# LemonATsu/DANBO-pytorch

Hardware: AMD Instinct MI355X
Metric: ray-samples/sec at 512x512x64 samples (higher is better)
Workload: dtype f32 (fp16x2-split MFMA products, fp32 accumulate); 1 GPU; H36M danbo_base network, 512x512 rays x (48 coarse + 16 importance) samples, 1 pose / 1 camera per rank, cylinder near/far, exact in-volume culling; rays=262144, samples_per_ray=64, parallelism=rays-dp1

## Files before the change

### danbo-pytorch_amd/core/_hip.py

```python
import ctypes
import os
import re
from ctypes import c_char_p, c_float, c_int, c_void_p
from types import SimpleNamespace

import torch

_HERE = os.path.dirname(os.path.abspath(__file__))
LIB_PATH = os.environ.get("DANBO_HIP_LIB") or os.path.join(os.path.dirname(_HERE), "libdanbo_hip.so")

P = c_void_p
I = c_int
F = c_float


class HeaderError(ValueError):
    """include/danbo_hip.h left the subset of C that parse_header reads"""


_SCALARS = {"int": c_int, "long": ctypes.c_long, "long long": ctypes.c_longlong, "size_t": ctypes.c_size_t, "float": c_float,
            **{f"{u}int{n}_t": getattr(ctypes, f"c_{u}int{n}") for u in ("", "u") for n in (8, 16, 32, 64)}}
_TAIL = r"((?:\*\s*(?:const\b\s*)?)*)(\w+)\s*(?:\[\s*(\w*)\s*\])?$"
_DECL = re.compile(r"(?:const\s+)?(long\s+long|\w+)\b\s*" + _TAIL)
_MORE = re.compile(_TAIL)
# ... 177 lines not shown
    _p_functions, _p_structs, _p_constants = parse_header(_f.read())
if _p_structs or _p_constants or set(_p_functions) & (set(_functions) | set(_r_functions)):
    raise HeaderError(f"{PARTMAP_HEADER_PATH} declares a struct, a constant, or a name another header declares")
PARTMAP_SIGNATURES = {name: argtypes for name, (_, argtypes) in _p_functions.items()}
PARTMAP_RESTYPES = {name: restype for name, (restype, _) in _p_functions.items()}

METRICS_HEADER_PATH = os.path.join(os.path.dirname(HEADER_PATH), "danbo_metrics.h")
if not os.path.exists(METRICS_HEADER_PATH):
    raise RuntimeError(f"{METRICS_HEADER_PATH} not found (the binding of the image metrics is derived from it, it lies beside danbo_hip.h)")
with open(METRICS_HEADER_PATH) as _f:
    _m_functions, _m_structs, _m_constants = parse_header(_f.read())
if _m_structs or _m_constants or set(_m_functions) & (set(_functions) | set(_r_functions) | set(_p_functions)):
    raise HeaderError(f"{METRICS_HEADER_PATH} declares a struct, a constant, or a name another header declares")
METRICS_SIGNATURES = {name: argtypes for name, (_, argtypes) in _m_functions.items()}
METRICS_RESTYPES = {name: restype for name, (restype, _) in _m_functions.items()}
ANERF_MAX_D = C.DANBO_ANERF_MAX_D

TRAIN_TENSORS = (
    ["graph_net.layers.0.lin.weight", "graph_net.layers.0.adj_w", "graph_net.layers.0.bias", "graph_net.layers.1.lin.weight",
     "graph_net.layers.1.adj_w", "graph_net.layers.1.bias", "graph_net.layers.2.weight", "graph_net.layers.2.bias",
     "graph_net.layers.3.weight", "graph_net.layers.3.bias", "graph_net.axis_scale",
     "prob_linears.layers.0.lin.weight", "prob_linears.layers.0.adj_w", "prob_linears.layers.0.bias", "prob_linears.layers.1.weight",
     "prob_linears.layers.1.bias", "prob_linears.layers.2.weight", "prob_linears.layers.2.bias"]
    + [f"pts_linears.{i}.weight" for i in range(8)] + [f"pts_linears.{i}.bias" for i in range(8)]
    + ["alpha_linear.weight", "alpha_linear.bias", "feature_linear.weight", "feature_linear.bias", "views_linears.0.weight",
       "views_linears.0.bias", "rgb_linear.weight", "rgb_linear.bias", "framecodes.codes.weight"])
N_TRAIN_TENSORS = C.DANBO_T_COUNT
_anchors = {"graph_net.axis_scale": C.DANBO_T_AXIS_SCALE, "prob_linears.layers.0.lin.weight": C.DANBO_T_A_W0,
            "pts_linears.0.weight": C.DANBO_T_PTS_W0, "pts_linears.0.bias": C.DANBO_T_PTS_B0, "alpha_linear.weight": C.DANBO_T_ALPHA_W,
            "framecodes.codes.weight": C.DANBO_T_CODES}
if len(TRAIN_TENSORS) != N_TRAIN_TENSORS or any(TRAIN_TENSORS.index(k) != i for k, i in _anchors.items()):
    raise HeaderError(f"TRAIN_TENSORS does not line up with enum DanboTrainTensor of {HEADER_PATH}")

_lib = None


def lib():
    global _lib
    if _lib is None:
        if not os.path.exists(LIB_PATH):
            raise RuntimeError(
                f"{LIB_PATH} not found: build it with `make -C danbo-pytorch_amd/csrc` "
                "(or __graft_entry__.build()).  There is no CPU / PyTorch fallback.")
        l = ctypes.CDLL(LIB_PATH)
        for name, argtypes in {**SIGNATURES, **RASTER_SIGNATURES, **PARTMAP_SIGNATURES, **METRICS_SIGNATURES}.items():
            fn = getattr(l, name)
            fn.argtypes = argtypes
            fn.restype = RESTYPES.get(name) or RASTER_RESTYPES.get(name) or PARTMAP_RESTYPES.get(name) or METRICS_RESTYPES[name]
        if l.danbo_abi_version() != C.DANBO_ABI_VERSION:
            raise RuntimeError(f"{LIB_PATH} has ABI version {l.danbo_abi_version()}, {HEADER_PATH} declares {C.DANBO_ABI_VERSION}: "
                               "the library is stale, rebuild it with `make -C danbo-pytorch_amd/csrc`")
        _lib = l
    return _lib


def ptr(t):
    return None if t is None else c_void_p(t.data_ptr())


def stream():
    return c_void_p(torch.cuda.current_stream().cuda_stream)


# ... 12 lines not shown
```

### danbo-pytorch_amd/core/hip_ops.py

```python
import ctypes

import torch

from . import _hip
from ._hip import call as _call, ptr as _p, stream as _stream

J = _hip.C.DANBO_J
VOL = _hip.C.DANBO_VOL
FEAT = _hip.C.DANBO_FEAT
RAY_FLAT_VMAX = _hip.C.DANBO_RAY_FLAT_VMAX
H_STRIDE = _hip.C.DANBO_H_STRIDE
MLP_PACKED_FLOATS = _hip.C.DANBO_MLP_PACKED_FLOATS
ASSIGN16_PACKED_BYTES = _hip.C.DANBO_ASSIGN16_PACKED_BYTES
MLP16_PACKED_BYTES = _hip.C.DANBO_MLP16_PACKED_BYTES
ANERF_ENC_FLOATS = _hip.C.DANBO_ANERF_ENC_FLOATS
LINEAR16_ENC_K = _hip.C.DANBO_LINEAR16_ENC_K
TRUNK_PACKED_BYTES = _hip.C.DANBO_TRUNK_PACKED_BYTES
TRUNK_PE_WIDTH = _hip.C.DANBO_TRUNK_PE_WIDTH
VIEW_W = 128


def _f32(t, name):
    if t is None:
        return None
# ... 78 lines not shown


def bone_cull(geo, compact=True, cnt=None):
    bits = torch.empty(geo.M, device=geo.device, dtype=torch.int32)
    lst = None
    if compact:
        lst = torch.empty(geo.M, device=geo.device, dtype=torch.int32)
        if cnt is None:
            cnt = torch.zeros(1, device=geo.device, dtype=torch.int32)
        assert cnt.dtype == torch.int32 and cnt.numel() == 1 and cnt.is_contiguous()
    else:
        cnt = None
    rm = tuple(geo.ray_mask) if geo.ray_mask is not None else (None, None, None)
    flat = rm[3] if len(rm) > 3 else None
    _call("danbo_bone_cull", *geo.head(), _p(rm[0]), _p(rm[1]), _p(rm[2]), _p(flat), _p(bits), _p(lst), _p(cnt), _stream())
    return bits, lst, cnt


def ray_bone_mask(rays_o, rays_d, skts, align, axis_scale, t_lo, t_hi, want_flat=False):
    rays_o, rays_d, skts = _f32(rays_o, "rays_o"), _f32(rays_d, "rays_d"), _f32(skts, "skts")
    t_lo, t_hi = _f32(t_lo, "t_lo").reshape(-1), _f32(t_hi, "t_hi").reshape(-1)
    R, G = rays_o.shape[0], skts.shape[0]
    assert t_lo.shape[0] == R and t_hi.shape[0] == R
    mask = torch.empty(R, device=rays_o.device, dtype=torch.int32)
    flat = torch.empty(R, device=rays_o.device, dtype=torch.int32) if want_flat else None
    _call("danbo_ray_bone_mask", _p(rays_o), _p(rays_d), _p(t_lo), _p(t_hi), R, G, _p(skts), _p(_f32(align, "align")),
          _p(_f32(axis_scale, "axis_scale")), _p(mask), _p(flat), _stream())
    return (mask, t_lo, t_hi, flat) if want_flat else (mask, t_lo, t_hi)


# ... 781 lines not shown
```

### danbo-pytorch_amd/core/render_engine.py

```python
import ctypes

import torch

from . import _hip
from . import hip_ops as ops


class RenderEngine:
    fuse_resample = False

    def _key(self):
        return tuple((k, v.data_ptr(), v._version) for k, v in sorted(self.p.items()))

    def _sampling(self, N_samples, N_importance):
        cfg = self.cfg
        return (N_samples or cfg["N_samples"], N_importance or cfg["N_importance"], cfg["density_scale"],
                ops.density_act(cfg.get("density_act")))

    @staticmethod
    def frame_result(out, out0):
        return dict(rgb_map=out["rgb_map"], disp_map=out["disp_map"], acc_map=out["acc_map"], alpha=out["alpha"],
                    T_i=out["weights"], rgb0=out0["rgb_map"], disp0=out0["disp_map"], acc0=out0["acc_map"],
                    alpha0=out0["alpha"])

# ... 59 lines not shown
    fuse_resample = True

    def __init__(self, cfg, params, align, buffers=None, mlp_mode="f16split"):
        self.cfg = cfg
        self.p = params
        self.align = align.float().contiguous()
        self._packed_key = None
        self.packed = self.wrt = self.empty_consts = None
        self.mean_code = None
        self.profile = None
        self.skip_flat_rays = True
        self.mlp_form = 32
        assert mlp_mode in ("f16split", "fp32")
        self.mlp_mode = mlp_mode
        self.group_rows = False

    def refresh(self):
        key = self._key()
        if key == self._packed_key and getattr(self, "_built_mode", None) == (self.mlp_mode, self.mlp_form):
            return
        p = self.p
        dev = p["alpha_linear.weight"].device
        q = self._equalized(p) if self.mlp_mode == "f16split" else p
        self.pts_w = [q[f"pts_linears.{i}.weight"] for i in range(8)]
        self.pts_b = [q[f"pts_linears.{i}.bias"].contiguous() for i in range(8)]
        self.packed, self.wrt = ops.mlp_pack(self.pts_w, q["feature_linear.weight"], q["views_linears.0.weight"])
        self.packed16, self.views_b16 = ops.mlp16_pack(self.pts_w, q["feature_linear.weight"],
                                                       q["feature_linear.bias"], q["views_linears.0.weight"],
                                                       q["views_linears.0.bias"], form=self.mlp_form)
        self.alpha_w = q["alpha_linear.weight"].reshape(-1).contiguous()
# ... 106 lines not shown
        self.refresh()
        return ops.pose_volumes(bones, self.gw, self.cfg["multires_graph"])

    def view_constants(self, rays_d, skts, cam_idx, ray_list=None, ray_count=None):
        self.refresh()
        cfg = self.cfg
        ray_mode = {"world": 0, "root_local": 1}[cfg["ray_tr_type"]]
        normalise = 1 if cfg["view_type"] == "relray" else 0
        return ops.view_consts(rays_d, skts, ray_mode, normalise, cfg["multires_views"], self.framecodes,
                               self.mean_code, cam_idx, self.wrt,
                               self.views_b16 if self.mlp_mode == "f16split" else self.views_b, self.rgb_w,
                               self.rgb_b, self.empty_consts, {16: 1, 32: 2}[self.mlp_form] if self.mlp_mode == "f16split" else 0,
                               self.code_table, ray_list, ray_count)

    def forward_samples(self, rays_o, rays_d, skts, bones, cam_idx=None, z=None, pts=None, dense=False,
                        want_confd=False, volumes=None, view=None, fill=True, ray_mask=None, count=None):
        self.refresh()
        geo = ops.Geometry(rays_o, rays_d, skts, self.align, self.axis_scale, z=z, pts=pts, ray_mask=ray_mask)
        vols = self.volumes(bones) if volumes is None else volumes
        cview, raw_empty = self.view_constants(geo.rays_d, geo.skts, cam_idx) if view is None else view
        S = geo.S
        bits, lst, cnt = ops.bone_cull(geo, compact=not dense, cnt=count)
        if lst is not None and self.mlp_mode == "f16split" and self.group_rows:
            ops.group_rows(bits, lst, cnt)
        if self.mlp_mode == "f16split":
            h, confd = ops.gather_assign_blend16(geo, vols, bits, self.aw, self.assign16, lst, cnt, geo.M, want_confd)
        else:
            h, confd = ops.gather_assign_blend(geo, vols, bits, self.aw, lst, cnt, geo.M, want_confd)
        raw = ops.fill_raw(raw_empty, S) if fill or dense else torch.empty(geo.R, S, 4, device=raw_empty.device)
        if self.profile is not None:
            e0, e1 = torch.cuda.Event(enable_timing=True), torch.cuda.Event(enable_timing=True)
            e0.record()
        self._mlp(h, S, cview, raw, lst, cnt, geo.M)
        if self.profile is not None:
            e1.record()
            self.profile.setdefault("k_pe_mlp", []).append((e0, e1, cnt if cnt is not None else geo.M))
        extras = dict(valid_bits=bits, list=lst, count=cnt, confd_rows=confd, h_rows=h, volumes=vols)
# ... 78 lines not shown
            ops.near_far_boxes(rays_o, rays_d, skts, self.align, self.axis_scale, near, far)
        return near, far

    def render(self, rays_o, rays_d, skts, bones, cyls, cam_idx=None, N_samples=None, N_importance=None,
               chunk=4096, near_far=None, dense=False, keep=False, part_map=None, part_valid_only=False):
        S, Sf, B, act = self._sampling(N_samples, N_importance)
        self.refresh()
        part = self._part_mode(part_map)
        if part and not self._part_exact_culled(act):
            dense = True
        fused = S <= 64 and Sf <= 64
        lazy = not dense and not keep
        flat_mode = (lazy and (fused or (S <= 256 and Sf <= 64)) and self.skip_flat_rays and self.flat_rays_ok
                     and act[0] == "relu")
        near, far = self.near_far(rays_o, rays_d, cyls, skts, 0.0, 1.0, chunk) if near_far is None else near_far
        z = ops.coarse_samples(near, far, S)
        ray_mask = None if dense else ops.ray_bone_mask(rays_o, rays_d, skts, self.align, self.axis_scale, near, far,
                                                        want_flat=flat_mode)
        counts = torch.zeros(3, device=rays_o.device, dtype=torch.int32)
        flat = None
        vols = self.volumes(bones)
        if flat_mode:
            flat = ops.flat_rays(ray_mask[1], ray_mask[3], S, Sf, want_weights=not fused or bool(part), cnt=counts[2:3])
            view = self.view_constants(rays_d, skts, cam_idx, flat["ray_list"], flat["ray_count"])
        else:
            view = self.view_constants(rays_d, skts, cam_idx)
        if ray_mask is not None:
            ray_mask = ray_mask[:3]
        raw, ex = self.forward_samples(rays_o, rays_d, skts, bones, cam_idx, z=z, dense=dense, volumes=vols, view=view,
                                       fill=not lazy, ray_mask=ray_mask, count=counts[0:1], want_confd=bool(part))
        if fused:
            out0, z_all, z_fine, order = ops.composite_importance(
                raw, z, rays_d, Sf, B, bits=ex["valid_bits"] if lazy else None, raw_empty=view[1] if lazy else None,
                want_weights=keep or bool(part), flat=flat, act=act)
        else:
            out0 = ops.composite(raw, z, rays_d, B, bits=ex["valid_bits"] if lazy else None, raw_empty=view[1] if lazy else None,
                                 flat=flat, act=act)
            z_all, z_fine, order = ops.importance_samples(z, out0["weights"], Sf, flat=flat)
        raw_f, ex_f = self.forward_samples(rays_o, rays_d, skts, bones, cam_idx, z=z_fine, dense=dense,
                                           volumes=vols, view=view, fill=not lazy,
                                           ray_mask=ray_mask, count=counts[1:2], want_confd=bool(part))
        out = ops.composite_merged(raw, raw_f, order, z_all, rays_d, B, bits_a=ex["valid_bits"] if lazy else None,
                                   bits_b=ex_f["valid_bits"] if lazy else None, raw_empty=view[1] if lazy else None,
                                   want_raw=keep, flat=flat, act=act)
        if part:
            col, cb = self._part_colors(ex, S, part, part_valid_only, dense)
            col_f, cb_f = self._part_colors(ex_f, Sf, part, part_valid_only, dense)
            ops.composite_colors(col, out0["weights"], bits_a=cb, flat=flat, out=out0["rgb_map"])
            ops.composite_colors(col, out["weights"], col_f, order, cb, cb_f, flat=flat, out=out["rgb_map"])
        ret = self.frame_result(out, out0)
        if keep:
            ret.update(near=near, far=far, z_coarse=z, raw_coarse=raw, weights_coarse=out0["weights"], z_fine=z_fine,
                       z_sorted=z_all, sorted_idxs=order, raw_fine=raw_f, raw_sorted=out.get("raw_sorted"),
                       count_coarse=ex["count"], count_fine=ex_f["count"], valid_bits=ex["valid_bits"])
            if part:
                ret.update(confd_coarse=ex["confd_rows"], confd_fine=ex_f["confd_rows"], list_coarse=ex["list"],
# ... 14 lines not shown
```

### danbo-pytorch_amd/csrc/k_frame.hip

```cpp
#include "common.hpp"

using namespace danbo;

namespace {
struct FrameBuffers {
    float *near, *far, *cyl_scratch, *z, *vol_scratch, *volumes, *cview, *raw_empty, *h, *raw_a, *raw_b, *z_fine, *z_sorted, *weights0;
    uint32_t *bits_a, *bits_b, *ray_mask, *ray_flat;
    int32_t *list, *count, *order, *ray_list;
};

FrameBuffers carve(Carver& c, int R, int G, int S, int Sf, int chunk, int Wg) {
    FrameBuffers b;
    const size_t M = (size_t)R * S, Mf = (size_t)R * Sf;
    b.near = c.take<float>(R);
    b.far = c.take<float>(R);
    b.cyl_scratch = c.take<float>(8 * (size_t)((R + chunk - 1) / chunk));
    b.z = c.take<float>(M);
    b.vol_scratch = c.take<float>(3 * (size_t)G * 24 * Wg);
    b.volumes = c.take<float>((size_t)G * 24 * 240);
    b.cview = c.take<float>((size_t)R * 128);
    b.raw_empty = c.take<float>((size_t)R * 4);
    b.ray_mask = c.take<uint32_t>(R);
    b.ray_flat = c.take<uint32_t>(R);
    b.ray_list = c.take<int32_t>(R);
// ... 25 lines not shown
    DANBO_CHECK_ARG(m && r && o && workspace && S >= 3 && S <= 256 && Sf >= 1 && Sf <= 64);
    DANBO_CHECK_ARG(r->R >= 1 && r->G >= 1 && r->R % r->G == 0 && r->chunk >= 1);
    DANBO_CHECK_ARG(r->rays_o && r->rays_d && r->skts && r->bones && r->cyls);
    DANBO_CHECK_ARG(o->rgb_map && o->disp_map && o->acc_map && o->alpha && o->weights && o->rgb0 && o->disp0 && o->acc0 && o->alpha0);
    const int R = r->R, G = r->G;
    const bool flat_rays = m->flat_rays_ok != 0 && act == DANBO_DENSITY_RELU;
    DANBO_CHECK_ARG(workspace_bytes >= danbo_render_frame_workspace(R, G, S, Sf, r->chunk, m->graph_width));
    Carver c(workspace);
    const FrameBuffers b = carve(c, R, G, S, Sf, r->chunk, m->graph_width);
    hipStream_t st = (hipStream_t)stream;

    DANBO_TRY(danbo_near_far_cylinder(r->rays_o, r->rays_d, r->cyls, R, G, 0.f, 1.f, r->near_in, r->far_in, r->chunk, b.cyl_scratch,
                                      b.near, b.far, stream));
    if (m->use_volume_near_far)
        DANBO_TRY(danbo_near_far_boxes(r->rays_o, r->rays_d, r->skts, m->align, m->axis_scale, R, G, b.near, b.far, stream));
    DANBO_TRY(danbo_coarse_samples(b.near, b.far, R, S, nullptr, b.z, stream));
    DANBO_TRY(danbo_ray_bone_mask(r->rays_o, r->rays_d, b.near, b.far, R, G, r->skts, m->align, m->axis_scale, b.ray_mask,
                                  flat_rays ? b.ray_flat : nullptr, stream));
    DANBO_TRY(danbo_pose_volumes_fwd(r->bones, G, m->L_graph, m->graph_width, m->g_w0, m->g_adjw0, m->g_b0, m->g_w1, m->g_adjw1, m->g_b1,
                                     m->g_w2, m->g_b2, m->g_w3, m->g_b3, b.vol_scratch, b.volumes, stream));
    zero_words(b.count, 4, nullptr, 0, st);
    auto view_consts = [&](const int32_t* ray_list, const int32_t* ray_count) -> int {
        return danbo_view_consts(r->rays_d, r->skts, R, G, m->ray_mode, m->normalise, m->L_view, m->framecodes, m->n_codes, m->code_size,
                                 m->mean_code, r->cam_idx, m->views_w_ray_t, m->views_b_eff, m->rgb_w, m->rgb_b, m->empty_consts, 2,
                                 m->code_table, ray_list, ray_count, b.cview, b.raw_empty, stream);
    };
    const int32_t *ray_list = nullptr, *ray_count = nullptr;
    if (flat_rays) {
        DANBO_TRY(danbo_flat_rays(b.near, b.ray_flat, R, S, Sf, o->rgb0, o->disp0, o->acc0, b.weights0, o->alpha0, b.z_fine, o->rgb_map,
                                  o->disp_map, o->acc_map, o->weights, o->alpha, b.ray_list, b.count + 3, 3, stream));
        ray_list = b.ray_list;
        ray_count = b.count + 3;
    }
    DANBO_TRY(view_consts(ray_list, ray_count));
    auto cull = [&](const float* zz, int s, uint32_t* bits, int32_t* count) -> int {
        DANBO_TRY(danbo_bone_cull(r->rays_o, r->rays_d, zz, nullptr, R, s, G, r->skts, m->align, m->axis_scale, b.ray_mask, b.near, b.far,
                                  nullptr, bits, b.list, count, stream));
        return 0;
    };
    auto network = [&](const float* zz, int s, uint32_t* bits, int32_t* count, float* raw) -> int {
        DANBO_TRY(danbo_gather_assign_blend16_fwd(r->rays_o, r->rays_d, zz, nullptr, R, s, G, r->skts, m->align, m->axis_scale, b.volumes,
                                                  bits, b.list, count, R * s, m->assign16, m->a_b0, m->a_b1, m->a_w2, m->a_b2, b.h,
                                                  nullptr, reinterpret_cast<uint32_t*>(b.count + 2), stream));
        return danbo_pe_mlp32_fwd(b.h, b.list, count, R * s, s, m->mlp16, m->pts_b, m->alpha_w, m->alpha_b, b.cview, m->rgb_w,
                                  m->rgb_b, raw, nullptr, stream);
    };
    DANBO_TRY(cull(b.z, S, b.bits_a, b.count));
    DANBO_TRY(network(b.z, S, b.bits_a, b.count, b.raw_a));
    if (S <= 64) {
        DANBO_TRY(danbo_composite_importance_pdf_fwd_act(b.raw_a, b.raw_empty, b.bits_a, b.z, r->rays_d, R, S, Sf, m->density_scale, nullptr,
// ... 26 lines not shown
```

### danbo-pytorch_amd/csrc/k_sample.hip

```cpp
#include "common.hpp"

namespace danbo {

__global__ __launch_bounds__(256) DANBO_NO_PK_F32 void k_cylinder_pass1(const float* __restrict__ rays_o,
                                                        const float* __restrict__ rays_d,
                                                        const float* __restrict__ cyl, int R, int G,
                                                        float near0, float far0,
                                                        const float* __restrict__ near_in,
                                                        const float* __restrict__ far_in, int chunk,
                                                        double* __restrict__ acc,
                                                        float* __restrict__ near_out,
                                                        float* __restrict__ far_out) {
    const int rays_per_pose = R / G;
    for (int r0 = blockIdx.x * blockDim.x; r0 < R; r0 += gridDim.x * blockDim.x) {
        const int r = r0 + threadIdx.x;
        const bool act = r < R;
        const int rc = act ? r : R - 1;
        const int g = min(rc / rays_per_pose, G - 1);
        float o[3] = {rays_o[3 * rc], rays_o[3 * rc + 1], rays_o[3 * rc + 2]};
        float d[3] = {rays_d[3 * rc], rays_d[3 * rc + 1], rays_d[3 * rc + 2]};
        float c[3] = {cyl[5 * g], cyl[5 * g + 1], cyl[5 * g + 2]};
        float nr, fr;
        const bool hit = cylinder_bounds(o, d, c, near_in ? near_in[rc] : near0, far_in ? far_in[rc] : far0, &nr, &fr) && act;
        if (act) {
// ... 131 lines not shown
        }
        int any = ok ? 1 : 0;
#pragma unroll
        for (int off = 16; off > 0; off >>= 1) {
            lo = fminf(lo, __shfl_xor(lo, off, 64));
            hi = fmaxf(hi, __shfl_xor(hi, off, 64));
            any |= __shfl_xor(any, off, 64);
        }
        if (j == 0 && r0 < R && any) {
            near_io[r] = lo;
            far_io[r] = hi;
        }
    }
}

__device__ __forceinline__ float coarse_sample(float n_, float f_, int s, int S, const float* __restrict__ t_rand, long m) {
    float v = coarse_z(n_, f_, s, S);
    if (t_rand) {
        const float zp = s > 0 ? coarse_z(n_, f_, s - 1, S) : v;
        const float zn = s + 1 < S ? coarse_z(n_, f_, s + 1, S) : v;
        const float lower = s > 0 ? mul_rn(0.5f, add_rn(v, zp)) : v;
        const float upper = s + 1 < S ? mul_rn(0.5f, add_rn(zn, v)) : v;
        v = add_rn(lower, mul_rn(sub_rn(upper, lower), t_rand[m]));
    }
    return v;
}

__global__ __launch_bounds__(256) void k_coarse_samples4(const float* __restrict__ nr, const float* __restrict__ fr,
                                                         int R, int S, const float* __restrict__ t_rand,
                                                         float4* __restrict__ z) {
    const unsigned S4 = (unsigned)S / 4u;
    const unsigned M4 = (unsigned)R * S4;
    for (unsigned q = blockIdx.x * blockDim.x + threadIdx.x; q < M4; q += gridDim.x * blockDim.x) {
        const unsigned r = q / S4;
        const int s0 = 4 * (int)(q - r * S4);
        const float n_ = nr[r], f_ = fr[r];
        const long m = 4L * q;
        float4 v;
        v.x = coarse_sample(n_, f_, s0, S, t_rand, m);
        v.y = coarse_sample(n_, f_, s0 + 1, S, t_rand, m + 1);
        v.z = coarse_sample(n_, f_, s0 + 2, S, t_rand, m + 2);
        v.w = coarse_sample(n_, f_, s0 + 3, S, t_rand, m + 3);
// ... 20 lines not shown
}

__device__ __forceinline__ void load_point(const float* __restrict__ rays_o, const float* __restrict__ rays_d,
                                           const float* __restrict__ z, const float* __restrict__ pts, long m, int S,
                                           float* p) {
    if (pts != nullptr) {
        p[0] = pts[3 * m]; p[1] = pts[3 * m + 1]; p[2] = pts[3 * m + 2];
    } else {
        const int r = (int)(m / S);
        const float o[3] = {rays_o[3 * r], rays_o[3 * r + 1], rays_o[3 * r + 2]};
        const float d[3] = {rays_d[3 * r], rays_d[3 * r + 1], rays_d[3 * r + 2]};
        sample_point(o, d, z[m], p);
    }
}

typedef float v2f __attribute__((ext_vector_type(2)));

template <int HI>
__device__ __forceinline__ v2f pk_mul_bcast(v2f m, v2f x) {
    v2f d;
    if (HI) asm("v_pk_mul_f32 %0, %1, %2 op_sel:[1,0] op_sel_hi:[1,1]" : "=v"(d) : "v"(m), "v"(x));
    else asm("v_pk_mul_f32 %0, %1, %2 op_sel:[0,0] op_sel_hi:[0,1]" : "=v"(d) : "v"(m), "v"(x));
    return d;
}
__device__ __forceinline__ v2f pk_add(v2f a, v2f b) {
    v2f d;
    asm("v_pk_add_f32 %0, %1, %2" : "=v"(d) : "v"(a), "v"(b));
    return d;
}
__device__ __forceinline__ v2f pk_add_bcast_hi(v2f m, v2f a) {
    v2f d;
    asm("v_pk_add_f32 %0, %1, %2 op_sel:[1,0] op_sel_hi:[1,1]" : "=v"(d) : "v"(m), "v"(a));
    return d;
}
__device__ __forceinline__ void affine_pk(const float* M, v2f x, v2f y, v2f z, v2f* q) {
#pragma unroll
    for (int k = 0; k < 3; ++k) {
        const float4 r = *reinterpret_cast<const float4*>(M + 4 * k);
        const v2f m01 = {r.x, r.y}, m23 = {r.z, r.w};
        v2f s = pk_add(pk_mul_bcast<0>(m01, x), pk_mul_bcast<1>(m01, y));
        s = pk_add(s, pk_mul_bcast<0>(m23, z));
        q[k] = pk_add_bcast_hi(m23, s);
    }
}

__device__ __forceinline__ bool segment_misses_bone(const float* sk, const float* al, const float* sc ,
                                                    const float* o, const float* d, float zl, float zh) {
    float ol[3], dl[3], t[3];
    bone_local(sk, al, o, ol);
    for (int k = 0; k < 3; ++k) t[k] = sk[4 * k] * d[0] + sk[4 * k + 1] * d[1] + sk[4 * k + 2] * d[2];
    for (int k = 0; k < 3; ++k) dl[k] = al[4 * k] * t[0] + al[4 * k + 1] * t[1] + al[4 * k + 2] * t[2];
    const float pad = 1e-4f * fmaxf(fabsf(zl), fabsf(zh)) + 1e-5f;
    float tmin = zl - pad, tmax = zh + pad;
    bool miss = false;
    for (int k = 0; k < 3; ++k) {
        const float s = sc[k] * 1.001f + 1e-4f;
        if (fabsf(dl[k]) < 1e-12f) {
            miss = miss || fabsf(ol[k]) > s;
        } else {
// ... 109 lines not shown
    const bool prefilter = pts == nullptr && ray_mask == nullptr && nrays <= CULL_MAX_RAYS;
    float zreg[CULL_SPT];
    if (pts == nullptr) {
#pragma unroll
        for (int k = 0; k < CULL_SPT; ++k) zreg[k] = z[min(base + k * CULL_BLOCK + threadIdx.x, M - 1)];
    }
    uint32_t pre[CULL_SPT];
    if (ray_mask != nullptr) {
        bool any = false;
#pragma unroll
        for (int k = 0; k < CULL_SPT; ++k) {
            pre[k] = 0u;
            if (base + k * CULL_BLOCK + threadIdx.x < M) {
                const int r = r_first + ray_of(off0 + k * CULL_BLOCK + threadIdx.x);
                const float lo = t_lo[r], hi = t_hi[r];
                const float slack = 5e-5f * fmaxf(fabsf(lo), fabsf(hi));
                const bool inside = zreg[k] >= lo - slack && zreg[k] <= hi + slack;
                pre[k] = inside ? ray_mask[r] : (1u << J) - 1u;
                if (!inside && ray_flat != nullptr) ray_flat[r] = 0u;
            }
            any = any || pre[k] != 0u;
        }
        if (!__syncthreads_or(any ? 1 : 0)) {
#pragma unroll
            for (int k = 0; k < CULL_SPT; ++k)
                if (base + k * CULL_BLOCK + threadIdx.x < M) valid_bits[base + k * CULL_BLOCK + threadIdx.x] = 0u;
            return;
        }
    }
    for (int i = threadIdx.x; i < J * 16; i += CULL_BLOCK) s_align[i] = align[i];
    for (int i = threadIdx.x; i < J * 4; i += CULL_BLOCK) s_scale[i] = (i & 3) < 3 ? fabsf(axis_scale[(i >> 2) * 3 + (i & 3)]) : 0.f;
// ... 55 lines not shown
            sample_point(oa, da, ma < M ? zreg[2 * pr] : z[M - 1], pa);
            sample_point(ob, db, mb < M ? zreg[2 * pr + 1] : z[M - 1], pb);
        }
        const int ga = pose_of(ra), gb = pose_of(rb);
        uint32_t ba = 0, bb = 0;
        uint32_t need = (1u << J) - 1u;
        if (ray_mask != nullptr) {
            need = wave_or(pre[2 * pr] | pre[2 * pr + 1]);
        } else if (prefilter) {
            uint32_t mine = s_mask[ra - r_first] | s_mask[rb - r_first];
            need = wave_or(mine);
        }
        if (__builtin_amdgcn_readfirstlane((int)__all(ga == gb))) {
            const v2f px = {pa[0], pb[0]}, py = {pa[1], pb[1]}, pz = {pa[2], pb[2]};
            const float* sk = s_skt + (ga - g0) * J * 16;
            while (need) {
                const int j = __builtin_ctz(need);
                need &= need - 1u;
                v2f l[3], t[3];
                affine_pk(sk + 16 * j, px, py, pz, l);
                affine_pk(s_align + 16 * j, l[0], l[1], l[2], t);
                const float* sc = s_scale + 4 * j;
                const bool ina = !(fabsf(t[0].x) > sc[0] || fabsf(t[1].x) > sc[1] || fabsf(t[2].x) > sc[2]);
                const bool inb = !(fabsf(t[0].y) > sc[0] || fabsf(t[1].y) > sc[1] || fabsf(t[2].y) > sc[2]);
                ba |= (ina ? 1u : 0u) << j;
                bb |= (inb ? 1u : 0u) << j;
            }
        } else {
            const float* ska = s_skt + (ga - g0) * J * 16;
            const float* skb = s_skt + (gb - g0) * J * 16;
            for (int j = 0; j < J; ++j) {
                float pt[3];
                bone_local(ska + 16 * j, s_align + 16 * j, pa, pt);
                ba |= (in_volume(pt, s_scale + 4 * j) ? 1u : 0u) << j;
                bone_local(skb + 16 * j, s_align + 16 * j, pb, pt);
                bb |= (in_volume(pt, s_scale + 4 * j) ? 1u : 0u) << j;
            }
        }
        bits4[2 * pr] = ma < M ? ba : 0u;
        bits4[2 * pr + 1] = mb < M ? bb : 0u;
        if (ma < M) valid_bits[ma] = ba;
        if (mb < M) valid_bits[mb] = bb;
// ... 927 lines not shown
```

### danbo-pytorch_amd/csrc/sample_math.hpp

```cpp
#pragma once
#include <math.h>
#include <stdint.h>

#if defined(__HIPCC__)
#define DANBO_HD __host__ __device__ __forceinline__
#else
#define DANBO_HD inline
#endif

namespace danbo {

constexpr int J = 24;
constexpr int FEAT = 15;
constexpr int VOXF = 5;
constexpr int VRES = 16;
constexpr int VOL = 240;

#if defined(__HIP_DEVICE_COMPILE__)
DANBO_HD float mul_rn(float a, float b) { return __fmul_rn(a, b); }
DANBO_HD float add_rn(float a, float b) { return __fadd_rn(a, b); }
DANBO_HD float sub_rn(float a, float b) { return __fsub_rn(a, b); }
DANBO_HD float div_rn(float a, float b) { return __fdiv_rn(a, b); }
DANBO_HD double dmul_rn(double a, double b) { return __dmul_rn(a, b); }
DANBO_HD double dadd_rn(double a, double b) { return __dadd_rn(a, b); }
// ... 6 lines not shown
DANBO_HD double dadd_rn(double a, double b) { volatile double r = a + b; return r; }
#endif

DANBO_HD float norm3_torch(float x, float y, float z) { return sqrtf(fmaf(z, z, fmaf(y, y, mul_rn(x, x)))); }
DANBO_HD float norm2_torch(float x, float y) { return sqrtf(fmaf(y, y, mul_rn(x, x))); }

DANBO_HD float linspace01(int i, int n) {
    if (n <= 1) return 0.f;
    const float step = div_rn(1.0f, (float)(n - 1));
    return (i < n / 2) ? mul_rn((float)i, step) : sub_rn(1.0f, mul_rn((float)(n - 1 - i), step));
}

DANBO_HD float coarse_z(float nr, float fr, int s, int S) {
    const float t = linspace01(s, S);
    return add_rn(mul_rn(nr, sub_rn(1.0f, t)), mul_rn(fr, t));
}

DANBO_HD void sample_point(const float* o, const float* d, float z, float* p) {
    p[0] = add_rn(o[0], mul_rn(d[0], z));
    p[1] = add_rn(o[1], mul_rn(d[1], z));
    p[2] = add_rn(o[2], mul_rn(d[2], z));
}

DANBO_HD void rotate_unfused(const float* M, const float* d, float* q) {
#pragma unroll
    for (int k = 0; k < 3; ++k) {
        const float* r = M + 4 * k;
        q[k] = add_rn(add_rn(mul_rn(r[0], d[0]), mul_rn(r[1], d[1])), mul_rn(r[2], d[2]));
    }
}
// ... 253 lines not shown
```

Measured before the change: 3.859 billion ray-samples/s.

## Cull only listed non-flat rays and fuse coarse sampling into the cull

Adds a bone-cull kernel that walks only the compacted list of non-flat rays instead of every ray-sample, and for the coarse pass also generates the z samples inline, so the separate coarse_samples launch is dropped. Per-ray origin, direction and mask data are staged in shared memory, and each workgroup compacts its output list with ballots and a single atomic. The aim is to avoid culling work on flat or empty rays and to save one full pass over z. The catch is that z is left uninitialised for unlisted rays, so downstream consumers must never read those entries. It applies only when there is a single pose and flat-ray mode is on.

```diff
diff --git a/danbo-pytorch_amd/core/_hip.py b/danbo-pytorch_amd/core/_hip.py
--- a/danbo-pytorch_amd/core/_hip.py
+++ b/danbo-pytorch_amd/core/_hip.py
@@ -215,6 +215,16 @@
     raise HeaderError(f"{METRICS_HEADER_PATH} declares a struct, a constant, or a name another header declares")
 METRICS_SIGNATURES = {name: argtypes for name, (_, argtypes) in _m_functions.items()}
 METRICS_RESTYPES = {name: restype for name, (restype, _) in _m_functions.items()}
+
+CULL_HEADER_PATH = os.path.join(os.path.dirname(HEADER_PATH), "danbo_cull.h")
+if not os.path.exists(CULL_HEADER_PATH):
+    raise RuntimeError(f"{CULL_HEADER_PATH} not found (the binding of the listed-ray cull is derived from it, it lies beside danbo_hip.h)")
+with open(CULL_HEADER_PATH) as _f:
+    _c_functions, _c_structs, _c_constants = parse_header(_f.read())
+if _c_structs or _c_constants or set(_c_functions) & (set(_functions) | set(_r_functions) | set(_p_functions) | set(_m_functions)):
+    raise HeaderError(f"{CULL_HEADER_PATH} declares a struct, a constant, or a name another header declares")
+CULL_SIGNATURES = {name: argtypes for name, (_, argtypes) in _c_functions.items()}
+CULL_RESTYPES = {name: restype for name, (restype, _) in _c_functions.items()}
 ANERF_MAX_D = C.DANBO_ANERF_MAX_D
 
 TRAIN_TENSORS = (
@@ -244,10 +254,11 @@
                 f"{LIB_PATH} not found: build it with `make -C danbo-pytorch_amd/csrc` "
                 "(or __graft_entry__.build()).  There is no CPU / PyTorch fallback.")
         l = ctypes.CDLL(LIB_PATH)
-        for name, argtypes in {**SIGNATURES, **RASTER_SIGNATURES, **PARTMAP_SIGNATURES, **METRICS_SIGNATURES}.items():
+        for name, argtypes in {**SIGNATURES, **RASTER_SIGNATURES, **PARTMAP_SIGNATURES, **METRICS_SIGNATURES, **CULL_SIGNATURES}.items():
             fn = getattr(l, name)
             fn.argtypes = argtypes
-            fn.restype = RESTYPES.get(name) or RASTER_RESTYPES.get(name) or PARTMAP_RESTYPES.get(name) or METRICS_RESTYPES[name]
+            fn.restype = (RESTYPES.get(name) or RASTER_RESTYPES.get(name) or PARTMAP_RESTYPES.get(name) or METRICS_RESTYPES.get(name)
+                          or CULL_RESTYPES[name])
         if l.danbo_abi_version() != C.DANBO_ABI_VERSION:
             raise RuntimeError(f"{LIB_PATH} has ABI version {l.danbo_abi_version()}, {HEADER_PATH} declares {C.DANBO_ABI_VERSION}: "
                                "the library is stale, rebuild it with `make -C danbo-pytorch_amd/csrc`")
diff --git a/danbo-pytorch_amd/core/hip_ops.py b/danbo-pytorch_amd/core/hip_ops.py
--- a/danbo-pytorch_amd/core/hip_ops.py
+++ b/danbo-pytorch_amd/core/hip_ops.py
@@ -116,6 +116,22 @@
     rm = tuple(geo.ray_mask) if geo.ray_mask is not None else (None, None, None)
     flat = rm[3] if len(rm) > 3 else None
     _call("danbo_bone_cull", *geo.head(), _p(rm[0]), _p(rm[1]), _p(rm[2]), _p(flat), _p(bits), _p(lst), _p(cnt), _stream())
+    return bits, lst, cnt
+
+
+def bone_cull_rays(geo, flat, bounds=None, cnt=None, rays_per_wg=0):
+    assert geo.z is not None and geo.ray_mask is not None and geo.z.is_contiguous()
+    bits = torch.empty(geo.M, device=geo.device, dtype=torch.int32)
+    lst = torch.empty(geo.M, device=geo.device, dtype=torch.int32)
+    if cnt is None:
+        cnt = torch.zeros(1, device=geo.device, dtype=torch.int32)
+    assert cnt.dtype == torch.int32 and cnt.numel() == 1 and cnt.is_contiguous()
+    near, far = (None, None) if bounds is None else (_f32(b, "bounds").reshape(-1) for b in bounds)
+    assert near is None or (near.shape[0] == geo.R and far.shape[0] == geo.R)
+    rm = tuple(geo.ray_mask)
+    _call("danbo_bone_cull_rays", *_ray_list(flat), _p(rm[0]), _p(rm[1]), _p(rm[2]), _p(geo.rays_o), _p(geo.rays_d), geo.R, geo.S,
+          geo.G, _p(geo.skts), _p(geo.align), _p(geo.axis_scale), _p(near), _p(far), _p(geo.z), int(rays_per_wg), _p(bits), _p(lst),
+          _p(cnt), _stream())
     return bits, lst, cnt
 
 
diff --git a/danbo-pytorch_amd/core/render_engine.py b/danbo-pytorch_amd/core/render_engine.py
--- a/danbo-pytorch_amd/core/render_engine.py
+++ b/danbo-pytorch_amd/core/render_engine.py
@@ -97,6 +97,7 @@
         assert mlp_mode in ("f16split", "fp32")
         self.mlp_mode = mlp_mode
         self.group_rows = False
+        self.cull_listed_rays = True
 
     def refresh(self):
         key = self._key()
@@ -233,13 +234,17 @@
                                self.code_table, ray_list, ray_count)
 
     def forward_samples(self, rays_o, rays_d, skts, bones, cam_idx=None, z=None, pts=None, dense=False,
-                        want_confd=False, volumes=None, view=None, fill=True, ray_mask=None, count=None):
+                        want_confd=False, volumes=None, view=None, fill=True, ray_mask=None, count=None, listed=None):
         self.refresh()
         geo = ops.Geometry(rays_o, rays_d, skts, self.align, self.axis_scale, z=z, pts=pts, ray_mask=ray_mask)
         vols = self.volumes(bones) if volumes is None else volumes
         cview, raw_empty = self.view_constants(geo.rays_d, geo.skts, cam_idx) if view is None else view
         S = geo.S
-        bits, lst, cnt = ops.bone_cull(geo, compact=not dense, cnt=count)
+        if listed is not None:
+            assert not dense and pts is None
+            bits, lst, cnt = ops.bone_cull_rays(geo, listed[0], listed[1], cnt=count)
+        else:
+            bits, lst, cnt = ops.bone_cull(geo, compact=not dense, cnt=count)
         if lst is not None and self.mlp_mode == "f16split" and self.group_rows:
             ops.group_rows(bits, lst, cnt)
         if self.mlp_mode == "f16split":
@@ -348,7 +353,8 @@
         flat_mode = (lazy and (fused or (S <= 256 and Sf <= 64)) and self.skip_flat_rays and self.flat_rays_ok
                      and act[0] == "relu")
         near, far = self.near_far(rays_o, rays_d, cyls, skts, 0.0, 1.0, chunk) if near_far is None else near_far
-        z = ops.coarse_samples(near, far, S)
+        listed_cull = flat_mode and self.cull_listed_rays and not part and skts.shape[0] == 1
+        z = torch.empty(rays_o.shape[0], S, device=rays_o.device, dtype=torch.float32) if listed_cull else ops.coarse_samples(near, far, S)
         ray_mask = None if dense else ops.ray_bone_mask(rays_o, rays_d, skts, self.align, self.axis_scale, near, far,
                                                         want_flat=flat_mode)
         counts = torch.zeros(3, device=rays_o.device, dtype=torch.int32)
@@ -362,7 +368,8 @@
         if ray_mask is not None:
             ray_mask = ray_mask[:3]
         raw, ex = self.forward_samples(rays_o, rays_d, skts, bones, cam_idx, z=z, dense=dense, volumes=vols, view=view,
-                                       fill=not lazy, ray_mask=ray_mask, count=counts[0:1], want_confd=bool(part))
+                                       fill=not lazy, ray_mask=ray_mask, count=counts[0:1], want_confd=bool(part),
+                                       listed=(flat, (near, far)) if listed_cull else None)
         if fused:
             out0, z_all, z_fine, order = ops.composite_importance(
                 raw, z, rays_d, Sf, B, bits=ex["valid_bits"] if lazy else None, raw_empty=view[1] if lazy else None,
@@ -373,7 +380,8 @@
             z_all, z_fine, order = ops.importance_samples(z, out0["weights"], Sf, flat=flat)
         raw_f, ex_f = self.forward_samples(rays_o, rays_d, skts, bones, cam_idx, z=z_fine, dense=dense,
                                            volumes=vols, view=view, fill=not lazy,
-                                           ray_mask=ray_mask, count=counts[1:2], want_confd=bool(part))
+                                           ray_mask=ray_mask, count=counts[1:2], want_confd=bool(part),
+                                           listed=(flat, None) if listed_cull else None)
         out = ops.composite_merged(raw, raw_f, order, z_all, rays_d, B, bits_a=ex["valid_bits"] if lazy else None,
                                    bits_b=ex_f["valid_bits"] if lazy else None, raw_empty=view[1] if lazy else None,
                                    want_raw=keep, flat=flat, act=act)
diff --git a/danbo-pytorch_amd/csrc/cull_math.hpp b/danbo-pytorch_amd/csrc/cull_math.hpp
--- /dev/null
+++ b/danbo-pytorch_amd/csrc/cull_math.hpp
@@ -0,0 +1,54 @@
+#pragma once
+#include "common.hpp"
+
+namespace danbo {
+
+typedef float v2f __attribute__((ext_vector_type(2)));
+
+template <int HI>
+__device__ __forceinline__ v2f pk_mul_bcast(v2f m, v2f x) {
+    v2f d;
+    if (HI) asm("v_pk_mul_f32 %0, %1, %2 op_sel:[1,0] op_sel_hi:[1,1]" : "=v"(d) : "v"(m), "v"(x));
+    else asm("v_pk_mul_f32 %0, %1, %2 op_sel:[0,0] op_sel_hi:[0,1]" : "=v"(d) : "v"(m), "v"(x));
+    return d;
+}
+__device__ __forceinline__ v2f pk_add(v2f a, v2f b) {
+    v2f d;
+    asm("v_pk_add_f32 %0, %1, %2" : "=v"(d) : "v"(a), "v"(b));
+    return d;
+}
+__device__ __forceinline__ v2f pk_add_bcast_hi(v2f m, v2f a) {
+    v2f d;
+    asm("v_pk_add_f32 %0, %1, %2 op_sel:[1,0] op_sel_hi:[1,1]" : "=v"(d) : "v"(m), "v"(a));
+    return d;
+}
+__device__ __forceinline__ void affine_pk(const float* M, v2f x, v2f y, v2f z, v2f* q) {
+#pragma unroll
+    for (int k = 0; k < 3; ++k) {
+        const float4 r = *reinterpret_cast<const float4*>(M + 4 * k);
+        const v2f m01 = {r.x, r.y}, m23 = {r.z, r.w};
+        v2f s = pk_add(pk_mul_bcast<0>(m01, x), pk_mul_bcast<1>(m01, y));
+        s = pk_add(s, pk_mul_bcast<0>(m23, z));
+        q[k] = pk_add_bcast_hi(m23, s);
+    }
+}
+
+__device__ __forceinline__ float mask_slack(float lo, float hi) { return 5e-5f * fmaxf(fabsf(lo), fabsf(hi)); }
+
+__device__ __forceinline__ void in_volume_pk(const float* sk, const float* s_align, const float* s_scale, uint32_t need,
+                                             v2f px, v2f py, v2f pz, uint32_t& ba, uint32_t& bb) {
+    while (need) {
+        const int j = __builtin_ctz(need);
+        need &= need - 1u;
+        v2f l[3], t[3];
+        affine_pk(sk + 16 * j, px, py, pz, l);
+        affine_pk(s_align + 16 * j, l[0], l[1], l[2], t);
+        const float* sc = s_scale + 4 * j;
+        const bool ina = !(fabsf(t[0].x) > sc[0] || fabsf(t[1].x) > sc[1] || fabsf(t[2].x) > sc[2]);
+        const bool inb = !(fabsf(t[0].y) > sc[0] || fabsf(t[1].y) > sc[1] || fabsf(t[2].y) > sc[2]);
+        ba |= (ina ? 1u : 0u) << j;
+        bb |= (inb ? 1u : 0u) << j;
+    }
+}
+
+}
diff --git a/danbo-pytorch_amd/csrc/k_cull_rays.hip b/danbo-pytorch_amd/csrc/k_cull_rays.hip
--- /dev/null
+++ b/danbo-pytorch_amd/csrc/k_cull_rays.hip
@@ -0,0 +1,163 @@
+#include "common.hpp"
+#include "../../include/danbo_cull.h"
+#include "cull_math.hpp"
+
+namespace danbo {
+
+constexpr int CR_BLOCK = 256;
+constexpr int CR_PAIR = 2 * CR_BLOCK;
+constexpr int CR_MAX_RPW = 384;
+constexpr int CR_MAX_SAMPLES = 16384;
+constexpr int CR_MAX_BALLOTS = CR_MAX_SAMPLES / 64;
+
+template <bool COARSE>
+__global__ __launch_bounds__(CR_BLOCK) void k_cull_rays(const int32_t* __restrict__ ray_list, const int32_t* __restrict__ ray_count,
+                                                        const uint32_t* __restrict__ ray_mask, const float* __restrict__ t_lo,
+                                                        const float* __restrict__ t_hi, const float* __restrict__ rays_o,
+                                                        const float* __restrict__ rays_d, const float* __restrict__ skts,
+                                                        const float* __restrict__ align, const float* __restrict__ axis_scale,
+                                                        const float* __restrict__ near, const float* __restrict__ far,
+                                                        float* __restrict__ z , int R, int S, int rpw,
+                                                        uint32_t* __restrict__ valid_bits, int32_t* __restrict__ list,
+                                                        int32_t* __restrict__ count) {
+    __shared__ __attribute__((aligned(16))) float s_align[J * 16];
+    __shared__ __attribute__((aligned(16))) float s_scale[J * 4];
+    __shared__ __attribute__((aligned(16))) float s_skt[J * 16];
+    __shared__ float4 s_o[CR_MAX_RPW];
+    __shared__ float4 s_d[CR_MAX_RPW];
+    __shared__ float4 s_m[CR_MAX_RPW];
+    __shared__ unsigned long long s_ball[CR_MAX_BALLOTS];
+    __shared__ int s_off[CR_MAX_BALLOTS];
+    __shared__ int s_base;
+
+    const int n = min(max(*ray_count, 0), R);
+    const int i0 = blockIdx.x * rpw;
+    if (i0 >= n) return;
+    const int nr = min(rpw, n - i0);
+    const int T = nr * S;
+    const int tid = threadIdx.x, lane = tid & 63, wave = tid >> 6;
+
+    for (int i = tid; i < nr; i += CR_BLOCK) {
+        const int r = min(max(ray_list[i0 + i], 0), R - 1);
+        const float lo = t_lo[r], hi = t_hi[r];
+        const float slack = mask_slack(lo, hi);
+        s_o[i] = make_float4(rays_o[3 * r], rays_o[3 * r + 1], rays_o[3 * r + 2], COARSE ? near[r] : 0.f);
+        s_d[i] = make_float4(rays_d[3 * r], rays_d[3 * r + 1], rays_d[3 * r + 2], COARSE ? far[r] : 0.f);
+        s_m[i] = make_float4(lo - slack, hi + slack, __builtin_bit_cast(float, ray_mask[r]), __builtin_bit_cast(float, r));
+    }
+    for (int i = tid; i < J * 16; i += CR_BLOCK) { s_align[i] = align[i]; s_skt[i] = skts[i]; }
+    for (int i = tid; i < J * 4; i += CR_BLOCK) s_scale[i] = (i & 3) < 3 ? fabsf(axis_scale[(i >> 2) * 3 + (i & 3)]) : 0.f;
+    __syncthreads();
+
+    const float inv_S = 1.0f / (float)S;
+    auto ray_of = [&](int li) {
+        int q = (int)((float)li * inv_S);
+        q -= (q * S > li) ? 1 : 0;
+        q += ((q + 1) * S <= li) ? 1 : 0;
+        return q;
+    };
+    const int nturns = (T + CR_PAIR - 1) / CR_PAIR;
+
+    for (int c = 0; c < nturns; ++c) {
+        const int la = c * CR_PAIR + tid, lb = la + CR_BLOCK;
+        const int lac = min(la, T - 1), lbc = min(lb, T - 1);
+        const int ia = ray_of(lac), ib = ray_of(lbc);
+        const int sa = lac - ia * S, sb = lbc - ib * S;
+        const float4 oa = s_o[ia], da = s_d[ia], qa = s_m[ia];
+        const float4 ob = s_o[ib], db = s_d[ib], qb = s_m[ib];
+        const size_t ma = (size_t)__builtin_bit_cast(int, qa.w) * S + sa, mb = (size_t)__builtin_bit_cast(int, qb.w) * S + sb;
+        float za, zb;
+        if (COARSE) {
+            za = coarse_sample(oa.w, da.w, sa, S, nullptr, 0);
+            zb = coarse_sample(ob.w, db.w, sb, S, nullptr, 0);
+            if (la < T) z[ma] = za;
+            if (lb < T) z[mb] = zb;
+        } else {
+            za = z[ma];
+            zb = z[mb];
+        }
+        const uint32_t pre_a = (za >= qa.x && za <= qa.y) ? __builtin_bit_cast(uint32_t, qa.z) : (1u << J) - 1u;
+        const uint32_t pre_b = (zb >= qb.x && zb <= qb.y) ? __builtin_bit_cast(uint32_t, qb.z) : (1u << J) - 1u;
+        const float o_a[3] = {oa.x, oa.y, oa.z}, d_a[3] = {da.x, da.y, da.z};
+        const float o_b[3] = {ob.x, ob.y, ob.z}, d_b[3] = {db.x, db.y, db.z};
+        float pa[3], pb[3];
+        sample_point(o_a, d_a, za, pa);
+        sample_point(o_b, d_b, zb, pb);
+        const v2f px = {pa[0], pb[0]}, py = {pa[1], pb[1]}, pz = {pa[2], pb[2]};
+        uint32_t ba = 0, bb = 0;
+        in_volume_pk(s_skt, s_align, s_scale, wave_or(pre_a | pre_b), px, py, pz, ba, bb);
+        if (la >= T) ba = 0u;
+        if (lb >= T) bb = 0u;
+        if (la < T) valid_bits[ma] = ba;
+        if (lb < T) valid_bits[mb] = bb;
+        const unsigned long long ball_a = __ballot(ba != 0u), ball_b = __ballot(bb != 0u);
+        if (lane == 0) {
+            s_ball[c * 8 + wave] = ball_a;
+            s_ball[c * 8 + 4 + wave] = ball_b;
+        }
+    }
+    __syncthreads();
+
+    const int nball = nturns * 8;
+    if (wave == 0) {
+        int run = 0;
+        for (int k0 = 0; k0 < nball; k0 += 64) {
+            const int k = k0 + lane;
+            const int cnt = k < nball ? (int)__popcll(s_ball[k]) : 0;
+            int incl = cnt;
+#pragma unroll
+            for (int off = 1; off < 64; off <<= 1) {
+                const int t = __shfl_up(incl, off, 64);
+                if (lane >= off) incl += t;
+            }
+            if (k < nball) s_off[k] = run + incl - cnt;
+            run += __builtin_amdgcn_readlane(incl, 63);
+        }
+        if (lane == 0) s_base = run > 0 ? atomicAdd(count, run) : 0;
+    }
+    __syncthreads();
+
+    const int base = s_base;
+    for (int c = 0; c < nturns; ++c) {
+#pragma unroll
+        for (int h = 0; h < 2; ++h) {
+            const int k = c * 8 + 4 * h + wave;
+            const unsigned long long ball = s_ball[k];
+            if ((ball >> lane) & 1ull) {
+                const int li = c * CR_PAIR + h * CR_BLOCK + tid;
+                const int i = ray_of(li);
+                const int r = __builtin_bit_cast(int, s_m[i].w);
+                list[base + s_off[k] + (int)__popcll(ball & ((1ull << lane) - 1ull))] = (int32_t)(r * S + (li - i * S));
+            }
+        }
+    }
+}
+
+}
+
+using namespace danbo;
+
+static int default_rays_per_wg(bool coarse) { return coarse ? 64 : 96; }
+
+extern "C" int danbo_bone_cull_rays(const int32_t* ray_list, const int32_t* ray_count, const uint32_t* ray_mask, const float* t_lo,
+                                    const float* t_hi, const float* rays_o, const float* rays_d, int R, int S, int G, const float* skts,
+                                    const float* align, const float* axis_scale, const float* near, const float* far, float* z,
+                                    int rays_per_wg, uint32_t* valid_bits, int32_t* list, int32_t* count, void* stream) {
+    DANBO_CHECK_ARG(ray_list && ray_count && ray_mask && t_lo && t_hi && rays_o && rays_d && skts && align && axis_scale);
+    DANBO_CHECK_ARG(z && valid_bits && list && count);
+    DANBO_CHECK_ARG((near == nullptr) == (far == nullptr));
+    DANBO_CHECK_ARG(G == 1);
+    DANBO_CHECK_ARG(R > 0 && S > 0 && S <= CR_MAX_SAMPLES && (long)R * S <= 0x7fffffffL);
+    DANBO_CHECK_ARG(rays_per_wg >= 0);
+    const bool coarse = near != nullptr;
+    int rpw = rays_per_wg > 0 ? rays_per_wg : default_rays_per_wg(coarse);
+    rpw = std::min(rpw, std::min(CR_MAX_RPW, CR_MAX_SAMPLES / S));
+    const int grid = ceil_div(R, rpw);
+    if (coarse)
+        hipLaunchKernelGGL(k_cull_rays<true>, dim3(grid), dim3(CR_BLOCK), 0, (hipStream_t)stream, ray_list, ray_count, ray_mask, t_lo,
+                           t_hi, rays_o, rays_d, skts, align, axis_scale, near, far, z, R, S, rpw, valid_bits, list, count);
+    else
+        hipLaunchKernelGGL(k_cull_rays<false>, dim3(grid), dim3(CR_BLOCK), 0, (hipStream_t)stream, ray_list, ray_count, ray_mask, t_lo,
+                           t_hi, rays_o, rays_d, skts, align, axis_scale, near, far, z, R, S, rpw, valid_bits, list, count);
+    DANBO_LAUNCH_RET();
+}
diff --git a/danbo-pytorch_amd/csrc/k_frame.hip b/danbo-pytorch_amd/csrc/k_frame.hip
--- a/danbo-pytorch_amd/csrc/k_frame.hip
+++ b/danbo-pytorch_amd/csrc/k_frame.hip
@@ -1,4 +1,5 @@
 #include "common.hpp"
+#include "../../include/danbo_cull.h"
 
 using namespace danbo;
 
@@ -63,7 +64,8 @@
                                       b.near, b.far, stream));
     if (m->use_volume_near_far)
         DANBO_TRY(danbo_near_far_boxes(r->rays_o, r->rays_d, r->skts, m->align, m->axis_scale, R, G, b.near, b.far, stream));
-    DANBO_TRY(danbo_coarse_samples(b.near, b.far, R, S, nullptr, b.z, stream));
+    const bool listed_cull = flat_rays && G == 1;
+    if (!listed_cull) DANBO_TRY(danbo_coarse_samples(b.near, b.far, R, S, nullptr, b.z, stream));
     DANBO_TRY(danbo_ray_bone_mask(r->rays_o, r->rays_d, b.near, b.far, R, G, r->skts, m->align, m->axis_scale, b.ray_mask,
                                   flat_rays ? b.ray_flat : nullptr, stream));
     DANBO_TRY(danbo_pose_volumes_fwd(r->bones, G, m->L_graph, m->graph_width, m->g_w0, m->g_adjw0, m->g_b0, m->g_w1, m->g_adjw1, m->g_b1,
@@ -82,7 +84,13 @@
         ray_count = b.count + 3;
     }
     DANBO_TRY(view_consts(ray_list, ray_count));
-    auto cull = [&](const float* zz, int s, uint32_t* bits, int32_t* count) -> int {
+    auto cull = [&](float* zz, int s, uint32_t* bits, int32_t* count) -> int {
+        if (listed_cull) {
+            const bool coarse = zz == b.z;
+            return danbo_bone_cull_rays(ray_list, ray_count, b.ray_mask, b.near, b.far, r->rays_o, r->rays_d, R, s, G, r->skts, m->align,
+                                        m->axis_scale, coarse ? b.near : nullptr, coarse ? b.far : nullptr, zz, 0, bits, b.list, count,
+                                        stream);
+        }
         DANBO_TRY(danbo_bone_cull(r->rays_o, r->rays_d, zz, nullptr, R, s, G, r->skts, m->align, m->axis_scale, b.ray_mask, b.near, b.far,
                                   nullptr, bits, b.list, count, stream));
         return 0;
diff --git a/danbo-pytorch_amd/csrc/k_sample.hip b/danbo-pytorch_amd/csrc/k_sample.hip
--- a/danbo-pytorch_amd/csrc/k_sample.hip
+++ b/danbo-pytorch_amd/csrc/k_sample.hip
@@ -1,4 +1,5 @@
 #include "common.hpp"
+#include "cull_math.hpp"
 
 namespace danbo {
 
@@ -169,18 +170,6 @@
     }
 }
 
-__device__ __forceinline__ float coarse_sample(float n_, float f_, int s, int S, const float* __restrict__ t_rand, long m) {
-    float v = coarse_z(n_, f_, s, S);
-    if (t_rand) {
-        const float zp = s > 0 ? coarse_z(n_, f_, s - 1, S) : v;
-        const float zn = s + 1 < S ? coarse_z(n_, f_, s + 1, S) : v;
-        const float lower = s > 0 ? mul_rn(0.5f, add_rn(v, zp)) : v;
-        const float upper = s + 1 < S ? mul_rn(0.5f, add_rn(zn, v)) : v;
-        v = add_rn(lower, mul_rn(sub_rn(upper, lower), t_rand[m]));
-    }
-    return v;
-}
-
 __global__ __launch_bounds__(256) void k_coarse_samples4(const float* __restrict__ nr, const float* __restrict__ fr,
                                                          int R, int S, const float* __restrict__ t_rand,
                                                          float4* __restrict__ z) {
@@ -231,35 +220,6 @@
     }
 }
 
-typedef float v2f __attribute__((ext_vector_type(2)));
-
-template <int HI>
-__device__ __forceinline__ v2f pk_mul_bcast(v2f m, v2f x) {
-    v2f d;
-    if (HI) asm("v_pk_mul_f32 %0, %1, %2 op_sel:[1,0] op_sel_hi:[1,1]" : "=v"(d) : "v"(m), "v"(x));
-    else asm("v_pk_mul_f32 %0, %1, %2 op_sel:[0,0] op_sel_hi:[0,1]" : "=v"(d) : "v"(m), "v"(x));
-    return d;
-}
-__device__ __forceinline__ v2f pk_add(v2f a, v2f b) {
-    v2f d;
-    asm("v_pk_add_f32 %0, %1, %2" : "=v"(d) : "v"(a), "v"(b));
-    return d;
-}
-__device__ __forceinline__ v2f pk_add_bcast_hi(v2f m, v2f a) {
-    v2f d;
-    asm("v_pk_add_f32 %0, %1, %2 op_sel:[1,0] op_sel_hi:[1,1]" : "=v"(d) : "v"(m), "v"(a));
-    return d;
-}
-__device__ __forceinline__ void affine_pk(const float* M, v2f x, v2f y, v2f z, v2f* q) {
-#pragma unroll
-    for (int k = 0; k < 3; ++k) {
-        const float4 r = *reinterpret_cast<const float4*>(M + 4 * k);
-        const v2f m01 = {r.x, r.y}, m23 = {r.z, r.w};
-        v2f s = pk_add(pk_mul_bcast<0>(m01, x), pk_mul_bcast<1>(m01, y));
-        s = pk_add(s, pk_mul_bcast<0>(m23, z));
-        q[k] = pk_add_bcast_hi(m23, s);
-    }
-}
 
 __device__ __forceinline__ bool segment_misses_bone(const float* sk, const float* al, const float* sc ,
                                                     const float* o, const float* d, float zl, float zh) {
@@ -399,7 +359,7 @@
             if (base + k * CULL_BLOCK + threadIdx.x < M) {
                 const int r = r_first + ray_of(off0 + k * CULL_BLOCK + threadIdx.x);
                 const float lo = t_lo[r], hi = t_hi[r];
-                const float slack = 5e-5f * fmaxf(fabsf(lo), fabsf(hi));
+                const float slack = mask_slack(lo, hi);
                 const bool inside = zreg[k] >= lo - slack && zreg[k] <= hi + slack;
                 pre[k] = inside ? ray_mask[r] : (1u << J) - 1u;
                 if (!inside && ray_flat != nullptr) ray_flat[r] = 0u;
@@ -485,18 +445,7 @@
         if (__builtin_amdgcn_readfirstlane((int)__all(ga == gb))) {
             const v2f px = {pa[0], pb[0]}, py = {pa[1], pb[1]}, pz = {pa[2], pb[2]};
             const float* sk = s_skt + (ga - g0) * J * 16;
-            while (need) {
-                const int j = __builtin_ctz(need);
-                need &= need - 1u;
-                v2f l[3], t[3];
-                affine_pk(sk + 16 * j, px, py, pz, l);
-                affine_pk(s_align + 16 * j, l[0], l[1], l[2], t);
-                const float* sc = s_scale + 4 * j;
-                const bool ina = !(fabsf(t[0].x) > sc[0] || fabsf(t[1].x) > sc[1] || fabsf(t[2].x) > sc[2]);
-                const bool inb = !(fabsf(t[0].y) > sc[0] || fabsf(t[1].y) > sc[1] || fabsf(t[2].y) > sc[2]);
-                ba |= (ina ? 1u : 0u) << j;
-                bb |= (inb ? 1u : 0u) << j;
-            }
+            in_volume_pk(sk, s_align, s_scale, need, px, py, pz, ba, bb);
         } else {
             const float* ska = s_skt + (ga - g0) * J * 16;
             const float* skb = s_skt + (gb - g0) * J * 16;
diff --git a/danbo-pytorch_amd/csrc/sample_math.hpp b/danbo-pytorch_amd/csrc/sample_math.hpp
--- a/danbo-pytorch_amd/csrc/sample_math.hpp
+++ b/danbo-pytorch_amd/csrc/sample_math.hpp
@@ -44,6 +44,18 @@
 DANBO_HD float coarse_z(float nr, float fr, int s, int S) {
     const float t = linspace01(s, S);
     return add_rn(mul_rn(nr, sub_rn(1.0f, t)), mul_rn(fr, t));
+}
+
+DANBO_HD float coarse_sample(float n_, float f_, int s, int S, const float* __restrict__ t_rand, long m) {
+    float v = coarse_z(n_, f_, s, S);
+    if (t_rand) {
+        const float zp = s > 0 ? coarse_z(n_, f_, s - 1, S) : v;
+        const float zn = s + 1 < S ? coarse_z(n_, f_, s + 1, S) : v;
+        const float lower = s > 0 ? mul_rn(0.5f, add_rn(v, zp)) : v;
+        const float upper = s + 1 < S ? mul_rn(0.5f, add_rn(zn, v)) : v;
+        v = add_rn(lower, mul_rn(sub_rn(upper, lower), t_rand[m]));
+    }
+    return v;
 }
 
 DANBO_HD void sample_point(const float* o, const float* d, float z, float* p) {
diff --git a/include/danbo_cull.h b/include/danbo_cull.h
--- /dev/null
+++ b/include/danbo_cull.h
@@ -0,0 +1,22 @@
+#ifndef DANBO_CULL_H
+#define DANBO_CULL_H
+
+#include <stddef.h>
+#include <stdint.h>
+
+#ifdef __cplusplus
+extern "C" {
+#endif
+
+int danbo_bone_cull_rays(const int32_t* ray_list, const int32_t* ray_count, const uint32_t* ray_mask ,
+                         const float* t_lo , const float* t_hi , const float* rays_o, const float* rays_d,
+                         int R, int S, int G, const float* skts , const float* align ,
+                         const float* axis_scale , const float* near , const float* far ,
+                         float* z , int rays_per_wg, uint32_t* valid_bits ,
+                         int32_t* list , int32_t* count , void* stream);
+
+#ifdef __cplusplus
+}
+#endif
+
+#endif
```

After: 3.916 billion ray-samples/s, median of 6. 1.01x the previous value.
